# OpenDriveLab/ViDAR

Measured on AMD Instinct MI355X. Metric: train samples/sec (6-cam->BEV step), higher is better.
Workload: dtype f32

## Files before the change

include/vidar_hip.h:

```cpp
#ifndef VIDAR_HIP_H_
#define VIDAR_HIP_H_

#include <stddef.h>
#include <stdint.h>

#ifdef __cplusplus
extern "C" {
#endif

#define VIDAR_ERR_BAD_ARG (-22)

int vidar_abi_version(void);
int vidar_marker(int id, void* stream);

int vidar_set_deterministic(int on);
int vidar_get_deterministic(void);

int vidar_dvr_max_d(void);

int vidar_dvr_render_forward_f32(const float* sigma, const float* origin, const float* points,
                                 const float* tindex, float* pred_dist ,
                                 float* gt_dist , int N, int M, int T, int TO, int Z, int Y,
                                 int X, int train_phase, void* stream);

int vidar_dvr_render_f32(const float* sigma, const float* origin, const float* points,
                         const float* tindex, float* pred_dist, float* gt_dist, float* grad_sigma,
                         int N, int M, int T, int TO, int Z, int Y, int X, int loss_type,
                         void* stream);

int vidar_dvr_init_f32(const float* points, const float* tindex, float* occupancy, int N, int M,
                       int T, int Z, int Y, int X, void* stream);

int vidar_dvxlr_max_d(void);


int vidar_dvr_set_sort_min_waves(int min_waves);
int vidar_dvr_set_traversal(int mode);
int vidar_dvxlr_set_pad_mode(int mode);

int vidar_dvxlr_render_f32(const float* sigma, const float* origin, const float* points,
                           const float* tindex, float* pred_dist, float* gt_dist, float* dd_dsigma,
                           float* indices, int N, int M, int T, int TO, int Z, int Y, int X,
                           void* stream);

size_t vidar_dvxlr_get_grad_sigma_workspace_bytes(int N, int T, int Z, int Y, int X, int volumes );
int vidar_dvxlr_get_grad_sigma_f32(const float* elementwise_mult ,
                                   const float* indices , const float* tindex,
                                   float* grad_sigma , int N, int M, int L, int T,
                                   int Z, int Y, int X, void* workspace, size_t workspace_bytes,
                                   void* stream);

int vidar_dvxlr2_render_f32(const float* sigma, const float* origin, const float* points,
                            const float* tindex, const float* sigma_regul, float* pred_dist,
                            float* gt_dist, float* dd_dsigma, float* indices, float* ray_pred,
                            float* indicator, int N, int M, int T, int TO, int Z, int Y, int X,
                            void* stream);

int vidar_dvxlr2_get_grad_sigma_f32(const float* elementwise_mult, const float* indices,
                                    const float* tindex, const float* indicator,
                                    const float* grad_ray_pred, float* grad_sigma,
                                    float* grad_sigma_regul, int N, int M, int L, int T, int Z, int Y,
                                    int X, void* workspace, size_t workspace_bytes, void* stream);

size_t vidar_knn1_d3_workspace_bytes(int N, int P1);
int vidar_knn1_d3_fwd(const float* p1, const float* p2, const int64_t* lengths1,
                      const int64_t* lengths2, int64_t* idx, float* dist2, void* workspace, int N,
                      int P1, int P2, void* stream);
int vidar_knn1_d3_bwd(const float* p1, const float* p2, const int64_t* lengths1,
                      const int64_t* lengths2, const int64_t* idx, const float* grad_dist2,
                      float* grad_p1, float* grad_p2, int N, int P1, int P2, void* stream);
int vidar_knn1_d3_bwd_workspace_bytes(int N, int P2, int64_t* bytes);
int vidar_knn1_d3_bwd_ws(const float* p1, const float* p2, const int64_t* lengths1,
                         const int64_t* lengths2, const int64_t* idx, const float* grad_dist2,
                         float* grad_p1, float* grad_p2, int N, int P1, int P2, void* workspace,
                         size_t workspace_bytes, void* stream);

int vidar_msda_fwd_f32(const float* value, const int64_t* spatial_shapes,
                       const int64_t* level_start_index, const float* sampling_loc,
                       const float* attn_weight, float* out, int B, int Nv, int H, int C, int Nq,
                       int L, int P, void* stream);
size_t vidar_msda_bwd_workspace_bytes(int B, int Nv, int H, int Nq, int L, int P);
int vidar_msda_set_item_order(int head_major);
int vidar_msda_bwd_f32(const float* value, const int64_t* spatial_shapes,
                       const int64_t* level_start_index, const float* sampling_loc,
                       const float* attn_weight, const float* grad_out, float* grad_value,
                       float* grad_sampling_loc, float* grad_attn_weight, int B, int Nv, int H, int C,
                       int Nq, int L, int P, void* workspace, size_t workspace_bytes, void* stream);

int vidar_msda_fused_fwd_f32(const float* value, const int64_t* spatial_shapes,
                             const int64_t* level_start_index, const float* off_raw, const float* logit_raw,
                             const float* ref, float* loc_out, float* w_out, float* out, int bs, int Qn, int Nv,
                             int H, int C, int Nq, int L, int P, int R, int mode, int merge_queue, void* stream);
int vidar_msda_fused_bwd_f32(const float* value, const int64_t* spatial_shapes,
                             const int64_t* level_start_index, const float* sampling_loc,
                             const float* attn_weight, const float* grad_out, float* grad_value,
                             float* grad_off_raw, float* grad_logit_raw, int bs, int Qn, int Nv, int H, int C,
                             int Nq, int L, int P, int merge_queue, void* workspace, size_t workspace_bytes, void* stream);

int vidar_drop_add_ln_fwd_f32(const float* x, const float* residual, const float* gamma, const float* beta, float* y,
                              float* sum_out, float* mean_out, float* rstd_out, int64_t rows, int C, float p, float eps,
                              uint32_t seed, void* stream);
int vidar_drop_add_ln_bwd_f32(const float* grad_y, const float* sum_in, const float* gamma, const float* mean_in,
                              const float* rstd_in, float* grad_x, float* grad_residual, float* grad_gamma,
                              float* grad_beta, void* workspace, int64_t rows, int C, float p, uint32_t seed,
                              void* stream);
size_t vidar_drop_add_ln_bwd_workspace_bytes(int64_t rows);

int vidar_relu_drop_fwd_f32(const float* x, float* y, int64_t n, float p, uint32_t seed, void* stream);
int vidar_relu_drop_bwd_f32(const float* grad_y, const float* y, float* grad_x, int64_t n, float p, void* stream);

int vidar_colsum_f32(const float* x, float* out, int64_t rows, int cols, void* stream);

int vidar_sca_plan_f32(const float* ref_3d, const float* lidar2img, float* ref_cam, uint8_t* bev_mask,
                       float* count, int64_t* idx, uint8_t* valid, int32_t* lens, int32_t* slot_of,
                       const float* pc_range, float img_h, float img_w, int F, int B, int N, int Q, int D,
                       void* stream);
int vidar_sca_rows_f32(const float* src, const int64_t* idx, const uint8_t* valid, const float* count, float* dst,
                       int B, int N, int S, int stride, int Q, int C, void* stream);
int vidar_sca_combine_f32(const float* src, const int32_t* slot_of, const float* count, float* dst, int B, int N,
                          int S, int Q, int C, void* stream);

size_t vidar_latent_render_bwd_workspace_bytes(int bs, int H, int W, int Z, int maps );
int vidar_latent_render_prob_fwd_f32(const float* occ, float* path_prob, int bs, int H, int W, int Z,
                                     int grid_num, float step, int act, void* stream);
int vidar_latent_render_prob_bwd_f32(const float* occ, const float* grad_path_prob, float* grad_occ,
                                     int bs, int H, int W, int Z, int grid_num, float step, int act,
                                     void* workspace, size_t workspace_bytes, void* stream);
int vidar_latent_render_gather_fwd_f32(const float* path_prob, const float* lora_a, float* feat,
                                       float* msum, int bs, int H, int W, int Z, int grid_num,
                                       float step, float eps, void* stream);
int vidar_latent_render_gather_bwd_f32(const float* path_prob, const float* lora_a, const float* feat,
                                       const float* msum, const float* grad_feat,
                                       float* grad_path_prob, float* grad_lora_a, int bs, int H,
                                       int W, int Z, int grid_num, float step, float eps,
                                       void* workspace, size_t workspace_bytes, void* stream);
int vidar_latent_render_gather_grouped_fwd_f32(const float* path_prob, const float* lora_a, float* feat, float* msum,
                                               int bs, int H, int W, int Z, int A, int grid_num, float step,
                                               float eps, void* stream);
int vidar_latent_render_gather_grouped_bwd_f32(const float* path_prob, const float* lora_a, const float* feat,
                                               const float* msum, const float* grad_feat, float* grad_path_prob,
                                               float* grad_lora_a, int bs, int H, int W, int Z, int A, int grid_num,
                                               float step, float eps, void* workspace, size_t workspace_bytes,
                                               void* stream);

size_t vidar_ray_bwd_workspace_bytes(int F, int Z, int Y, int X);
int vidar_ray_ce_fwd_f32(const float* sigma, const float* origin, const float* gt_pts,
                         const float* tindex, float* ce, float* lse, float* valid, int F, int R,
                         int Z, int Y, int X, int K, float step, void* stream);
int vidar_ray_ce_bwd_f32(const float* sigma, const float* origin, const float* gt_pts,
                         const float* tindex, const float* lse, const float* grad_ce,
                         float* grad_sigma, int F, int R, int Z, int Y, int X, int K, float step,
                         void* workspace, size_t workspace_bytes, void* stream);
int vidar_ray_gumbel_fwd_f32(const float* sigma, const float* origin, const float* pts,
                             const float* tindex, const float* noise , float* dist,
                             float* aux , int F, int R, int Z, int Y, int X, int K,
                             float step, void* stream);
int vidar_ray_gumbel_bwd_f32(const float* sigma, const float* origin, const float* pts,
                             const float* tindex, const float* aux, const float* grad_dist,
                             float* grad_sigma, int F, int R, int Z, int Y, int X, int K, float step,
                             void* workspace, size_t workspace_bytes, void* stream);
int vidar_ray_argmax_f32(const float* sigma, const float* origin, const float* pts,
                         const float* tindex, float* pred_dist, float* gt_dist, int F, int R, int Z,
                         int Y, int X, int K, float step, void* stream);
int vidar_ray_dist_fwd_f32(const float* sigma, const float* origin, const float* gt_pts,
                           const float* tindex, const float* noise , float* dist,
                           float* gt_len, float* aux , float* valid, int F, int R, int Z,
                           int Y, int X, int K, float step, void* stream);
int vidar_ray_dist_bwd_f32(const float* sigma, const float* origin, const float* gt_pts,
                           const float* tindex, const float* aux, const float* grad_dist,
                           float* grad_sigma, int F, int R, int Z, int Y, int X, int K, float step,
                           void* workspace, size_t workspace_bytes, void* stream);
int vidar_ray_max_k(void);
int vidar_ray_force_streamed(int on);

#define VIDAR_GEMM_F32 0
#define VIDAR_GEMM_BF16X3 1
#define VIDAR_GEMM_K_MAJOR 0
#define VIDAR_GEMM_MN_MAJOR 1
int vidar_gemm_f32(const float* A, int64_t lda, int a_layout, const float* B, int64_t ldb, int b_layout, float* C,
                   int64_t ldc, int M, int N, int K, int batch, int64_t strideA, int64_t strideB, int64_t strideC,
                   const float* scale, const float* shift, int vec_axis, const float* residual, int64_t ldr,
                   int64_t strideR, int relu, int precision, int reduce, float* a_rowsum, void* workspace,
                   size_t workspace_bytes, void* stream);
int vidar_gemm_splits(int M, int N, int K, int batch, int precision, int reduce);
size_t vidar_gemm_workspace_bytes(int M, int N, int K, int batch, int precision, int reduce);
int vidar_gemm_set_variant(int variant);

int vidar_dcn_set_variant(int variant);
int vidar_dcn_im2col_f32(const float* x, const float* offset, const float* mask, float* cols, int N,
                         int C, int H, int W, int Ho, int Wo, int kh, int kw, int stride, int pad,
                         int dil, void* stream);
int vidar_dcn_col2im_det_workspace_bytes(int N, int C, int H, int W, int64_t* bytes);
int vidar_dcn_col2im_f32(const float* grad_cols, const float* x, const float* offset,
                         const float* mask, float* grad_x, float* grad_offset, float* grad_mask,
                         int N, int C, int H, int W, int Ho, int Wo, int kh, int kw, int stride,
                         int pad, int dil, void* workspace, size_t workspace_bytes, void* stream);
size_t vidar_dcn_col2im_workspace_bytes(int N, int H, int W, int Ho, int Wo, int kh, int kw);

size_t vidar_conv3x3_few_workspace_bytes(int C);
int vidar_conv3x3_few_f32(const float* x, const float* weight, const float* bias, float* out, int N, int C, int H, int W,
                          int Cout, void* workspace, size_t workspace_bytes, void* stream);

int vidar_affine_act_fwd_f32(const float* x, const float* scale, const float* shift,
                             const float* residual, float* y, int N, int C, int HW, int relu,
                             void* stream);
int vidar_stem_bn_relu_pool_f32(const float* x, const float* scale, const float* shift, float* y, int N, int C,
                                int H, int W, void* stream);
int vidar_affine_act_bwd_f32(const float* grad_y, const float* y, const float* scale, float* grad_x,
                             float* grad_residual, int N, int C, int HW, int relu, void* stream);

int vidar_dcnv3_set_variant(int variant);
int vidar_dcnv3_forward_f32(const float* input, const float* offset, const float* mask, float* out, int N, int H, int W,
                            int kh, int kw, int stride_h, int stride_w, int pad_h, int pad_w, int dil_h, int dil_w,
                            int group, int group_channels, float offset_scale, void* stream);
size_t vidar_dcnv3_backward_workspace_bytes(int N, int H, int W, int kh, int kw, int stride_h, int stride_w, int pad_h,
                                            int pad_w, int dil_h, int dil_w, int group, int group_channels);
int vidar_dcnv3_backward_f32(const float* input, const float* offset, const float* mask, const float* grad_out,
                             float* grad_input, float* grad_offset, float* grad_mask, int N, int H, int W, int kh, int kw,
                             int stride_h, int stride_w, int pad_h, int pad_w, int dil_h, int dil_w, int group,
                             int group_channels, float offset_scale, void* workspace, size_t workspace_bytes, void* stream);

int vidar_det_match_cost_f32(const float* cls, const float* box, const float* gt_box_norm, const int32_t* gt_label,
                             const int32_t* gt_start, float* cost, float alpha, float gamma, float cls_weight,
                             float reg_weight, int NL, int B, int Q, int C, int total_g, void* stream);
size_t vidar_det_loss_workspace_bytes(int NL, int B, int Q);
int vidar_det_loss_fwd_f32(const float* cls, const float* box, const int32_t* labels, const int32_t* matched_gt,
                           const float* gt_box_norm, const int32_t* gt_start, const float* code_weights, float* sums,
                           float alpha, float gamma, int NL, int B, int Q, int C, int total_g, void* workspace,
                           size_t workspace_bytes, void* stream);
int vidar_det_loss_bwd_f32(const float* cls, const float* box, const int32_t* labels, const int32_t* matched_gt,
                           const float* gt_box_norm, const int32_t* gt_start, const float* code_weights,
                           const float* grad_sums, float* grad_cls, float* grad_box, float alpha, float gamma, int NL,
                           int B, int Q, int C, int total_g, void* stream);

int vidar_det_assign_workspace_bytes(int NL, int B, int Q, int total_g, int64_t* bytes);
int vidar_det_assign_f32(const float* cost, const int32_t* gt_start, int32_t* matched, int32_t* status, int NL, int B,
                         int Q, int total_g, void* workspace, size_t workspace_bytes, void* stream);

int vidar_det_eval_match_f32(const float* pred_box, const int32_t* pred_attr, const int32_t* pred_start,
                             const float* gt_box, const int32_t* gt_attr, const int32_t* gt_start, const float* dist_ths,
                             int32_t* match, int32_t* gt_match, float* err, int P, int G, int NS, int NT, int tp_index,
                             int num_classes, int barrier_class, void* stream);

int vidar_ray_eval_workspace_bytes(int P, int64_t* bytes);
int vidar_ray_eval_f64(const float* pred, const int32_t* pred_start, const float* gt, const int32_t* gt_start,
                       const float* origin, void* partial, int32_t* nn_idx, void* ray_err, void* interp, int P, int G,
                       int S, int max_gt, void* workspace, size_t workspace_bytes, void* stream);

#define VIDAR_IMG_PHOTO_FLOATS 12
int vidar_img_photometric_u8(const uint8_t* src, const float* photo, uint8_t* dst, int n, int H, int W, void* stream);
int vidar_img_photometric_f32(const uint8_t* src, const float* photo, float* dst, int n, int H, int W, void* stream);
size_t vidar_img_resample_workspace_bytes(int n, int crop_h, int out_w);
int vidar_img_resample_u8(const uint8_t* src, uint8_t* dst, int n, int H, int W, int crop_x, int crop_y, int crop_w,
                          int crop_h, int out_w, int out_h, const int32_t* tab_x, int ksize_x, const int32_t* tab_y,
                          int ksize_y, int flip, void* workspace, size_t workspace_bytes, void* stream);
int vidar_img_normalise_f32(const uint8_t* src, const float* photo, float* dst, int n, int H, int W, int out_h, int out_w,
                            int Hp, int Wp, const float* mean, const float* stdv, int to_rgb, void* stream);

#ifdef __cplusplus
}
#endif
#endif
```

vidar_amd/_lib.py:

```python
from __future__ import annotations

import ctypes
import os
from pathlib import Path

_PKG = Path(__file__).resolve().parent
LIB_PATH = _PKG / "libvidar_hip.so"
_lib = None
BAD_ARG = -22


class VidarHipError(RuntimeError):
    pass


def lib() -> ctypes.CDLL:
    global _lib
    if _lib is None:
        import torch
        if not LIB_PATH.exists():
            raise VidarHipError(
                f"{LIB_PATH} not found: build it with `python -m vidar_amd.build` "
                f"(or __graft_entry__.build()); vidar_amd has no CPU fallback")
        _lib = declare(ctypes.CDLL(str(LIB_PATH)))
        dcn = os.environ.get("VIDAR_DCN_VARIANT")
        if dcn is not None:
            _lib.vidar_dcn_set_variant(int(dcn))
        v3 = os.environ.get("VIDAR_DCNV3_VARIANT")
        if v3 is not None:
            _lib.vidar_dcnv3_set_variant(int(v3))
        order = os.environ.get("VIDAR_MSDA_ITEM_ORDER")
        if order is not None:
            _lib.vidar_msda_set_item_order(int(order))
    return _lib


_KIND = {"p": ctypes.c_void_p, "i": ctypes.c_int, "l": ctypes.c_int64, "z": ctypes.c_size_t, "f": ctypes.c_float,
         "u": ctypes.c_uint32}
_ABI = {
    "vidar_abi_version": "i",
    "vidar_marker": "i i p",
    "vidar_set_deterministic": "i i",
    "vidar_get_deterministic": "i",
    "vidar_dvr_max_d": "i",
    "vidar_dvr_render_forward_f32": "i 6p 8i p",
    "vidar_dvr_render_f32": "i 7p 8i p",
    "vidar_dvr_init_f32": "i 3p 6i p",
    "vidar_dvxlr_max_d": "i",
    "vidar_dvr_set_sort_min_waves": "i i",
    "vidar_dvr_set_traversal": "i i",
    "vidar_dvxlr_set_pad_mode": "i i",
    "vidar_dvxlr_render_f32": "i 8p 7i p",
    "vidar_dvxlr_get_grad_sigma_workspace_bytes": "z 6i",
    "vidar_dvxlr_get_grad_sigma_f32": "i 4p 7i p z p",
    "vidar_dvxlr2_render_f32": "i 11p 7i p",
    "vidar_dvxlr2_get_grad_sigma_f32": "i 7p 7i p z p",
    "vidar_knn1_d3_workspace_bytes": "z 2i",
    "vidar_knn1_d3_fwd": "i 7p 3i p",
    "vidar_knn1_d3_bwd": "i 8p 3i p",
    "vidar_knn1_d3_bwd_workspace_bytes": "i 2i p",
    "vidar_knn1_d3_bwd_ws": "i 8p 3i p z p",
    "vidar_msda_fwd_f32": "i 6p 7i p",
    "vidar_msda_bwd_workspace_bytes": "z 6i",
    "vidar_msda_set_item_order": "i i",
    "vidar_msda_bwd_f32": "i 9p 7i p z p",
    "vidar_msda_fused_fwd_f32": "i 9p 11i p",
    "vidar_msda_fused_bwd_f32": "i 9p 9i p z p",
    "vidar_drop_add_ln_fwd_f32": "i 8p l i 2f u p",
    "vidar_drop_add_ln_bwd_f32": "i 10p l i f u p",
    "vidar_drop_add_ln_bwd_workspace_bytes": "z l",
    "vidar_relu_drop_fwd_f32": "i 2p l f u p",
    "vidar_relu_drop_bwd_f32": "i 3p l f p",
    "vidar_colsum_f32": "i 2p l i p",
    "vidar_sca_plan_f32": "i 10p 2f 5i p",
    "vidar_sca_rows_f32": "i 5p 6i p",
    "vidar_sca_combine_f32": "i 4p 5i p",
    "vidar_latent_render_bwd_workspace_bytes": "z 5i",
    "vidar_latent_render_prob_fwd_f32": "i 2p 5i f i p",
    "vidar_latent_render_prob_bwd_f32": "i 3p 5i f i p z p",
    "vidar_latent_render_gather_fwd_f32": "i 4p 5i 2f p",
    "vidar_latent_render_gather_bwd_f32": "i 7p 5i 2f p z p",
    "vidar_latent_render_gather_grouped_fwd_f32": "i 4p 6i 2f p",
    "vidar_latent_render_gather_grouped_bwd_f32": "i 7p 6i 2f p z p",
    "vidar_ray_bwd_workspace_bytes": "z 4i",
    "vidar_ray_ce_fwd_f32": "i 7p 6i f p",
    "vidar_ray_ce_bwd_f32": "i 7p 6i f p z p",
    "vidar_ray_gumbel_fwd_f32": "i 7p 6i f p",
    "vidar_ray_gumbel_bwd_f32": "i 7p 6i f p z p",
    "vidar_ray_argmax_f32": "i 6p 6i f p",
    "vidar_ray_dist_fwd_f32": "i 9p 6i f p",
    "vidar_ray_dist_bwd_f32": "i 7p 6i f p z p",
    "vidar_ray_max_k": "i",
    "vidar_ray_force_streamed": "i i",
    "vidar_gemm_f32": "i p l i p l i p l 4i 3l 2p i p 2l 3i 2p z p",
    "vidar_gemm_splits": "i 6i",
    "vidar_gemm_workspace_bytes": "z 6i",
    "vidar_gemm_set_variant": "i i",
    "vidar_dcn_set_variant": "i i",
    "vidar_dcn_im2col_f32": "i 4p 11i p",
    "vidar_dcn_col2im_f32": "i 7p 11i p z p",
    "vidar_dcn_col2im_workspace_bytes": "z 7i",
    "vidar_dcn_col2im_det_workspace_bytes": "i 4i p",
    "vidar_conv3x3_few_workspace_bytes": "z i",
    "vidar_conv3x3_few_f32": "i 4p 5i p z p",
    "vidar_affine_act_fwd_f32": "i 5p 4i p",
    "vidar_stem_bn_relu_pool_f32": "i 4p 4i p",
    "vidar_affine_act_bwd_f32": "i 5p 4i p",
    "vidar_dcnv3_set_variant": "i i",
    "vidar_dcnv3_forward_f32": "i 4p 13i f p",
    "vidar_dcnv3_backward_workspace_bytes": "z 13i",
    "vidar_dcnv3_backward_f32": "i 7p 13i f p z p",
    "vidar_det_match_cost_f32": "i 6p 4f 5i p",
    "vidar_det_loss_workspace_bytes": "z 3i",
    "vidar_det_loss_fwd_f32": "i 8p 2f 5i p z p",
    "vidar_det_loss_bwd_f32": "i 10p 2f 5i p",
    "vidar_det_assign_workspace_bytes": "i 4i p",
    "vidar_det_assign_f32": "i 4p 4i p z p",
    "vidar_det_eval_match_f32": "i 10p 7i p",
    "vidar_ray_eval_workspace_bytes": "i i p",
    "vidar_ray_eval_f64": "i 9p 4i p z p",
    "vidar_img_photometric_u8": "i 3p 3i p",
    "vidar_img_photometric_f32": "i 3p 3i p",
    "vidar_img_resample_workspace_bytes": "z 3i",
    "vidar_img_resample_u8": "i 2p 9i p i p 2i p z p",
    "vidar_img_normalise_f32": "i 3p 7i 2p i p",
}


def signature(name):
    ret, *runs = _ABI[name].split()
    return _KIND[ret], [_KIND[r[-1]] for r in runs for _ in range(int(r[:-1] or 1))]


def declare(cdll):
    for name in _ABI:
        try:
            fn = getattr(cdll, name)
        except AttributeError:
            raise VidarHipError(f"{name} is not exported by {cdll._name}: rebuild the library") from None
        fn.restype, fn.argtypes = signature(name)
    return cdll


def check(rc: int, what: str):
    if rc == 0:
        return
    if rc == BAD_ARG:
        raise ValueError(f"{what}: invalid argument")
    raise VidarHipError(f"{what}: HIP error {rc}")


def ptr(t):
    return None if t is None else t.data_ptr()


def workspace(nbytes_fn, *dims, like):
    import torch
    n = nbytes_fn(*dims)
    if n == 0:
        return None, None, 0
    ws = torch.empty(n, dtype=torch.uint8, device=like.device)
    return ws, ptr(ws), n


def stream_of(t):
    import torch
    return torch.cuda.current_stream(t.device).cuda_stream


class OpTimer:
    def __init__(self):
        self.enabled = False
        self.records = {}

    def reset(self):
        self.records = {}

    class _Span:
        __slots__ = ("t", "name", "nbytes", "e0")

        def __init__(self, t, name, nbytes):
            self.t, self.name, self.nbytes = t, name, nbytes

        def __enter__(self):
            import torch
            self.e0 = torch.cuda.Event(enable_timing=True)
            self.e0.record()

        def __exit__(self, *exc):
            import torch
            e1 = torch.cuda.Event(enable_timing=True)
            e1.record()
            self.t.records.setdefault(self.name, []).append((self.e0, e1, self.nbytes))

    class _Null:
        def __enter__(self): return None
        def __exit__(self, *exc): return False

    _null = _Null()

    def span(self, name, nbytes=0):
        return OpTimer._Span(self, name, nbytes) if self.enabled else OpTimer._null

    def summary(self):
        import torch
        torch.cuda.synchronize()
        out = {}
        for name, recs in self.records.items():
            ms = [a.elapsed_time(b) for a, b, _ in recs]
            out[name] = dict(calls=len(ms), total_ms=sum(ms), avg_ms=sum(ms) / len(ms),
                             bytes_per_call=sum(r[2] for r in recs) / len(recs))
        return out


TIMER = OpTimer()
```

vidar_amd/plugin/backbones.py:

```python
from __future__ import annotations

import ctypes
import math
import os

import torch
import torch.nn as nn
import torch.nn.functional as F
from torch.autograd import Function
from torch.autograd.function import once_differentiable

from .registry import BACKBONES, NECKS
from .._lib import lib, check, ptr, stream_of, workspace, TIMER
from .. import gemm as G
from .. import deterministic


def dcn_col2im(grad_cols, x, offset, mask, kh, kw, stride, pad, dil, Ho, Wo, gather=True):
    N, C, H, W = x.shape
    gx = torch.empty_like(x); goff = torch.empty_like(offset); gm = torch.empty_like(mask)
    if deterministic.sync():
        nbytes = ctypes.c_int64(0)
        check(lib().vidar_dcn_col2im_det_workspace_bytes(N, C, H, W, ctypes.addressof(nbytes)), "dcn_col2im")
        nbytes = nbytes.value
        ws = torch.empty(nbytes, dtype=torch.uint8, device=x.device)
        ws_ptr = ptr(ws)
    else:
        ws, ws_ptr, nbytes = workspace(lib().vidar_dcn_col2im_workspace_bytes, N, H, W, Ho, Wo, kh, kw, like=x) \
            if gather else (None, None, 0)
    with TIMER.span("dcn_col2im", 4 * (3 * x.numel() + 2 * offset.numel() + 2 * mask.numel() + grad_cols.numel())):
        check(lib().vidar_dcn_col2im_f32(ptr(grad_cols), ptr(x), ptr(offset), ptr(mask), ptr(gx), ptr(goff), ptr(gm),
                                         N, C, H, W, Ho, Wo, kh, kw, stride, pad, dil, ws_ptr, nbytes, stream_of(x)),
              "dcn_col2im")
    return gx, goff, gm


class _ModulatedDeformConv(Function):

    @staticmethod
    def forward(ctx, x, offset, mask, weight, bias, stride, pad, dil, gemm_mode="lib", scale=None, shift=None,
                relu=False):
        x, offset, mask = x.float().contiguous(), offset.float().contiguous(), mask.float().contiguous()
        N, C, H, W = x.shape
        Cout, _, kh, kw = weight.shape
        Ho = (H + 2 * pad - dil * (kh - 1) - 1) // stride + 1
        Wo = (W + 2 * pad - dil * (kw - 1) - 1) // stride + 1
        cols = torch.empty((N, C * kh * kw, Ho * Wo), device=x.device)
        with TIMER.span("dcn_im2col", 4 * (x.numel() + offset.numel() + mask.numel() + cols.numel())):
            check(lib().vidar_dcn_im2col_f32(ptr(x), ptr(offset), ptr(mask), ptr(cols), N, C, H, W, Ho,
                                             Wo, kh, kw, stride, pad, dil, stream_of(x)), "dcn_im2col")
        fused = scale is not None
        if gemm_mode == "lib":
            assert not fused
            out = torch.bmm(weight.reshape(1, Cout, -1).expand(N, -1, -1), cols)
            if bias is not None:
                out = out + bias.view(1, -1, 1)
        else:
            sh = shift
            if bias is not None:
                sh = bias.float() if not fused else (shift + bias.float() * scale)
            out = G.conv_forward(weight.reshape(Cout, -1), cols, scale, sh, None, relu, G.precision_of(gemm_mode))
        ctx.save_for_backward(x, offset, mask, weight, cols, scale, out if (fused and relu) else None)
        ctx.cfg = (stride, pad, dil, Ho, Wo, bias is not None, gemm_mode, fused, relu)
        return out.view(N, Cout, Ho, Wo)

    @staticmethod
    @once_differentiable
    def backward(ctx, grad_out):
        x, offset, mask, weight, cols, scale, y = ctx.saved_tensors
        stride, pad, dil, Ho, Wo, has_bias, gemm_mode, fused, relu = ctx.cfg
        N, C, H, W = x.shape
        Cout, _, kh, kw = weight.shape
        go = grad_out.float().contiguous().view(N, Cout, Ho * Wo)
        if fused:
            go = _affine_act_backward(go, y if relu else go, scale, relu, False)[0]
        if gemm_mode == "lib":
            grad_weight = torch.bmm(go, cols.transpose(1, 2)).sum(0).reshape(weight.shape)
            grad_cols = torch.bmm(weight.reshape(1, Cout, -1).transpose(1, 2).expand(N, -1, -1), go)
        else:
            prec = G.precision_of(gemm_mode)
            grad_weight = G.conv_grad_weight(go, cols, prec).reshape(weight.shape) if ctx.needs_input_grad[3] else None
            grad_cols = G.conv_grad_input(weight.reshape(Cout, -1), go, prec)
        gx, goff, gm = dcn_col2im(grad_cols, x, offset, mask, kh, kw, stride, pad, dil, Ho, Wo)
        return (gx, goff, gm, grad_weight, (go.sum((0, 2)) if has_bias else None), None, None, None, None, None, None,
                None)


def modulated_deform_conv2d(x, offset, mask, weight, bias=None, stride=1, padding=0, dilation=1, bn=None, relu=False):
    m = G.mode() if (x.is_cuda and G.own_kernels()) else "lib"
    scale = shift = None
    if bn is not None:
        assert m != "lib"
        scale, shift = bn._scale_shift()
    return _ModulatedDeformConv.apply(x, offset, mask, weight, bias, int(stride), int(padding), int(dilation), m,
                                      scale, shift, bool(relu))


_CONV_OFFSET_OWN = os.environ.get("VIDAR_CONV_OFFSET", "lib") == "own"


class _Conv3x3Few(Function):

    @staticmethod
    def forward(ctx, x, weight, bias):
        x = x.contiguous()
        w = weight.contiguous()
        N, C, H, W = x.shape
        Cout = w.shape[0]
        out = torch.empty((N, Cout, H, W), device=x.device, dtype=torch.float32)
        ws, ws_ptr, ws_bytes = workspace(lib().vidar_conv3x3_few_workspace_bytes, C, like=x)
        with TIMER.span("conv3x3_few", 4 * (x.numel() + out.numel())):
            check(lib().vidar_conv3x3_few_f32(ptr(x), ptr(w), ptr(bias), ptr(out), N, C, H, W, Cout, ws_ptr, ws_bytes,
                                              stream_of(x)), "conv3x3_few")
        ctx.save_for_backward(x, w)
        ctx.has_bias = bias is not None
        return out

    @staticmethod
    @once_differentiable
    def backward(ctx, g):
        x, w = ctx.saved_tensors
        need = [ctx.needs_input_grad[0], ctx.needs_input_grad[1], ctx.has_bias and ctx.needs_input_grad[2]]
        gx, gw, gb = torch.ops.aten.convolution_backward(g.contiguous(), x, w, [w.shape[0]] if ctx.has_bias else None,
                                                         [1, 1], [1, 1], [1, 1], False, [0, 0], 1, need)
        return gx, gw, gb


def conv3x3_few_ok(conv, x):
    return (_CONV_OFFSET_OWN and x.is_cuda and x.dtype == torch.float32 and conv.weight.dtype == torch.float32
            and not torch.is_autocast_enabled() and x.dim() == 4
            and conv.kernel_size == (3, 3) and conv.stride == (1, 1) and conv.padding == (1, 1) and conv.dilation == (1, 1)
            and conv.groups == 1 and conv.padding_mode == "zeros" and conv.out_channels <= 32 and conv.in_channels % 8 == 0
            and x.shape[3] <= 191 and x.shape[2] * x.shape[3] < (1 << 30) and x.numel() > 0)


class ModulatedDeformConv2dPack(nn.Module):

    def __init__(self, in_channels, out_channels, kernel_size, stride=1, padding=0, dilation=1,
                 groups=1, deform_groups=1, bias=True):
        super().__init__()
        if groups != 1 or deform_groups != 1:
            raise NotImplementedError("DCNv2 kernels are built for groups == deform_groups == 1")
        k = kernel_size
        self.stride, self.padding, self.dilation, self.k = stride, padding, dilation, k
        self.weight = nn.Parameter(torch.empty(out_channels, in_channels, k, k))
        self.bias = nn.Parameter(torch.zeros(out_channels)) if bias else None
        n = in_channels * k * k
        nn.init.uniform_(self.weight, -1.0 / math.sqrt(n), 1.0 / math.sqrt(n))
        self.conv_offset = nn.Conv2d(in_channels, 3 * k * k, k, stride, padding, dilation, bias=True)
        nn.init.zeros_(self.conv_offset.weight)
        nn.init.zeros_(self.conv_offset.bias)

    def forward(self, x, bn=None, relu=False):
        if conv3x3_few_ok(self.conv_offset, x):
            out = _Conv3x3Few.apply(x, self.conv_offset.weight, self.conv_offset.bias)
        else:
            out = self.conv_offset(x)
        o1, o2, mask = torch.chunk(out, 3, dim=1)
        offset = torch.cat((o1, o2), dim=1)
        fuse = dict(bn=bn, relu=relu) if bn is not None else {}
        return modulated_deform_conv2d(x, offset, torch.sigmoid(mask), self.weight, self.bias,
                                       self.stride, self.padding, self.dilation, **fuse)


class _AffineAct(Function):

    @staticmethod
    def forward(ctx, x, scale, shift, residual, relu):
        x = x.float().contiguous()
        N, C, H, W = x.shape
        res = residual.float().contiguous() if residual is not None else None
        y = torch.empty_like(x)
        with TIMER.span("affine_act_fwd", 4 * x.numel() * (3 if res is not None else 2)):
            check(lib().vidar_affine_act_fwd_f32(ptr(x), ptr(scale), ptr(shift), ptr(res), ptr(y), N, C,
                                                 H * W, int(relu), stream_of(x)), "affine_act_fwd")
        ctx.save_for_backward(y, scale)
        ctx.cfg = (relu, residual is not None)
        return y

    @staticmethod
    @once_differentiable
    def backward(ctx, gy):
        y, scale = ctx.saved_tensors
        relu, has_res = ctx.cfg
        gx, gres = _affine_act_backward(gy.float().contiguous(), y, scale, relu, has_res)
        return gx, None, None, gres, None


def _affine_act_backward(gy, y, scale, relu, has_res):
    N, C = y.shape[:2]
    HW = y.numel() // (N * C)
    gx = torch.empty_like(y)
    gres = torch.empty_like(y) if has_res else None
    with TIMER.span("affine_act_bwd", 4 * y.numel() * (4 if has_res else 3)):
        check(lib().vidar_affine_act_bwd_f32(ptr(gy), ptr(y), ptr(scale), ptr(gx), ptr(gres), N, C,
                                             HW, int(relu), stream_of(y)), "affine_act_bwd")
    return gx, gres


class FrozenBN(nn.BatchNorm2d):

    def __init__(self, c, requires_grad=False):
        super().__init__(c)
        for p in self.parameters():
            p.requires_grad = requires_grad
        self._cache = None

    def _scale_shift(self):
        key = (self.weight._version, self.bias._version, self.running_mean._version,
               self.running_var._version, self.weight.device)
        if self._cache is None or self._cache[0] != key:
            with torch.no_grad():
                scale = (self.weight / torch.sqrt(self.running_var + self.eps)).float().contiguous()
                shift = (self.bias - self.running_mean * scale).float().contiguous()
            self._cache = (key, scale, shift)
        return self._cache[1], self._cache[2]

    def forward(self, x, residual=None, relu=False):
        if self.weight.requires_grad or not x.is_cuda:
            y = F.batch_norm(x, self.running_mean, self.running_var, self.weight, self.bias, False, 0.0,
                             self.eps)
            if residual is not None:
                y = y + residual
            return F.relu(y, inplace=True) if relu else y
        scale, shift = self._scale_shift()
        return _AffineAct.apply(x, scale, shift, residual, relu)


def stem_bn_relu_pool(x, bn):
    if not x.is_cuda or bn.weight.requires_grad or (torch.is_grad_enabled() and x.requires_grad):
        return None
    x = x.float().contiguous()
    N, C, H, W = x.shape
    if W % 4 or N * C > 65535:
        return None
    scale, shift = bn._scale_shift()
    y = torch.empty((N, C, (H - 1) // 2 + 1, W // 2), device=x.device, dtype=torch.float32)
    with TIMER.span("stem_bn_relu_pool", 4 * (x.numel() + y.numel())):
        check(lib().vidar_stem_bn_relu_pool_f32(ptr(x), ptr(scale), ptr(shift), ptr(y), N, C, H, W, stream_of(x)),
              "stem_bn_relu_pool")
    return y


class Conv1x1(nn.Conv2d):
    as_gemm = os.environ.get("VIDAR_CONV1X1_GEMM", "1") != "0"
    any_device = False

    def gemm_form(self, x):
        return (self.as_gemm and (x.is_cuda or self.any_device) and self.kernel_size == (1, 1) and self.padding == (0, 0)
                and self.groups == 1)

    def forward(self, x, presampled=False):
        if not self.gemm_form(x):
            assert not presampled
            return super().forward(x)
        if self.stride != (1, 1) and not presampled:
            x = x[:, :, ::self.stride[0], ::self.stride[1]].contiguous()
        N, C, H, W = x.shape
        out = torch.bmm(self.weight.view(1, self.out_channels, C).expand(N, -1, -1), x.reshape(N, C, H * W))
        if self.bias is not None:
            out = out + self.bias.view(1, -1, 1)
        return out.view(N, self.out_channels, H, W)


_AUTO_FUSE_RES = os.environ.get("VIDAR_AUTO_FUSE_RES", "1") != "0"


class _Conv1x1Identity(Function):

    @staticmethod
    def forward(ctx, x, weight):
        N, C, H, W = x.shape
        Cout = weight.shape[0]
        out = torch.bmm(weight.view(1, Cout, C).expand(N, -1, -1), x.reshape(N, C, H * W))
        ctx.save_for_backward(x, weight)
        return out.view(N, Cout, H, W), x.view_as(x)

    @staticmethod
    @once_differentiable
    def backward(ctx, g_out, g_ident):
        x, weight = ctx.saved_tensors
        N, C, H, W = x.shape
        Cout = weight.shape[0]
        gx = gw = None
        if g_out is None:
            return g_ident, None
        go = g_out.contiguous().view(N, Cout, H * W)
        if ctx.needs_input_grad[0]:
            wt = weight.view(1, Cout, C).transpose(1, 2).expand(N, -1, -1)
            if g_ident is not None:
                gx = g_ident.contiguous().view(N, C, H * W).baddbmm_(wt, go).view(N, C, H, W)
            else:
                gx = torch.bmm(wt, go).view(N, C, H, W)
        if ctx.needs_input_grad[1]:
            gw = torch.bmm(go, x.reshape(N, C, H * W).transpose(1, 2)).sum(0).view_as(weight)
        return gx, gw


_SHORTCUT_ACCUMULATE = os.environ.get("VIDAR_SHORTCUT_ACCUMULATE", "1") != "0"


def conv1x1_with_identity_ok(conv, x):
    return (_SHORTCUT_ACCUMULATE and isinstance(conv, Conv1x1) and conv.gemm_form(x) and conv.stride == (1, 1)
            and conv.bias is None and x.dtype == torch.float32 and conv.weight.dtype == torch.float32
            and x.requires_grad and torch.is_grad_enabled() and not torch.is_autocast_enabled() and x.is_contiguous())


class _Conv1x1BNAct(Function):

    @staticmethod
    def forward(ctx, x, weight, scale, shift, residual, relu, precision):
        x = x.float().contiguous()
        N, C, H, W = x.shape
        Cout = weight.shape[0]
        res = residual.float().contiguous().view(N, Cout, H * W) if residual is not None else None
        y = G.conv_forward(weight.reshape(Cout, C), x.view(N, C, H * W), scale, shift, res, relu, precision)
        ctx.save_for_backward(x, weight, scale, y if relu else None)
        ctx.cfg = (relu, residual is not None, precision)
        return y.view(N, Cout, H, W)

    @staticmethod
    @once_differentiable
    def backward(ctx, gy):
        x, weight, scale, y = ctx.saved_tensors
        relu, has_res, precision = ctx.cfg
        N, C, H, W = x.shape
        Cout = weight.shape[0]
        gy = gy.float().contiguous().view(N, Cout, H * W)
        gz, gres = _affine_act_backward(gy, y if relu else gy, scale, relu, has_res)
        gx = G.conv_grad_input(weight.reshape(Cout, C), gz, precision).view(N, C, H, W) if ctx.needs_input_grad[0] else None
        gw = G.conv_grad_weight(gz, x.view(N, C, H * W), precision).view_as(weight) if ctx.needs_input_grad[1] else None
        return gx, gw, None, None, (gres.view(N, Cout, H, W) if has_res else None), None, None


def _fuses_1x1(conv, bn, x, residual, hw, m):
    fuse = G.own_kernels(m) or (m == "auto" and residual is not None and _AUTO_FUSE_RES)
    in_range = 0 < hw < (1 << 22) and max(conv.in_channels, conv.out_channels) * hw < (1 << 29)
    return (fuse and x.is_cuda and not bn.weight.requires_grad and conv.bias is None and conv.kernel_size == (1, 1)
            and conv.padding == (0, 0) and conv.groups == 1 and in_range)


def conv1x1_bn_act(conv, bn, x, residual=None, relu=False, presampled=False):
    if presampled:
        return _conv1x1_bn_act_presampled(conv, bn, x, residual, relu)
    m = G.mode()
    hw = ((x.shape[2] - 1) // conv.stride[0] + 1) * ((x.shape[3] - 1) // conv.stride[1] + 1) if x.dim() == 4 else 0
    if not _fuses_1x1(conv, bn, x, residual, hw, m):
        return bn(conv(x), residual=residual, relu=relu)
    if conv.stride != (1, 1):
        x = x[:, :, ::conv.stride[0], ::conv.stride[1]]
    scale, shift = bn._scale_shift()
    return _Conv1x1BNAct.apply(x, conv.weight, scale, shift, residual, bool(relu), G.precision_of(m))


def _conv1x1_bn_act_presampled(conv, bn, xs, residual, relu):
    m = G.mode()
    if not _fuses_1x1(conv, bn, xs, residual, xs.shape[2] * xs.shape[3] if xs.dim() == 4 else 0, m):
        return bn(conv(xs, presampled=True), residual=residual, relu=relu)
    scale, shift = bn._scale_shift()
    return _Conv1x1BNAct.apply(xs, conv.weight, scale, shift, residual, bool(relu), G.precision_of(m))


_SHARE_SUBSAMPLE = os.environ.get("VIDAR_SHARE_SUBSAMPLE", "1") != "0"


class Bottleneck(nn.Module):
    expansion = 4

    def __init__(self, inplanes, planes, stride=1, downsample=None, style="caffe", dcn=None, bn_grad=False):
        super().__init__()
        s1, s2 = (stride, 1) if style == "caffe" else (1, stride)
        self.conv1 = Conv1x1(inplanes, planes, 1, stride=s1, bias=False)
        self.bn1 = FrozenBN(planes, bn_grad)
        if dcn is not None:
            self.conv2 = ModulatedDeformConv2dPack(planes, planes, 3, stride=s2, padding=1, dilation=1,
                                                   deform_groups=dcn.get("deform_groups", 1), bias=False)
        else:
            self.conv2 = nn.Conv2d(planes, planes, 3, stride=s2, padding=1, bias=False)
        self.bn2 = FrozenBN(planes, bn_grad)
        self.conv3 = Conv1x1(planes, planes * 4, 1, bias=False)
        self.bn3 = FrozenBN(planes * 4, bn_grad)
        self.downsample = downsample

    def _shares_subsample(self, x):
        d = self.downsample
        return (_SHARE_SUBSAMPLE and d is not None and len(d) == 2 and isinstance(d[0], Conv1x1) and isinstance(d[1], FrozenBN)
                and self.conv1.stride != (1, 1) and d[0].stride == self.conv1.stride
                and self.conv1.gemm_form(x) and d[0].gemm_form(x))

    def forward(self, x):
        if self._shares_subsample(x):
            sh, sw = self.conv1.stride
            xs = x[:, :, ::sh, ::sw].contiguous()
            identity = conv1x1_bn_act(self.downsample[0], self.downsample[1], xs, presampled=True)
            out = conv1x1_bn_act(self.conv1, self.bn1, xs, relu=True, presampled=True)
            return self._tail(out, identity)
        if self.downsample is None:
            identity = x
            if conv1x1_with_identity_ok(self.conv1, x) and not _fuses_1x1(self.conv1, self.bn1, x, None,
                                                                            x.shape[2] * x.shape[3], G.mode()):
                out, identity = _Conv1x1Identity.apply(x, self.conv1.weight)
                return self._tail(self.bn1(out, relu=True), identity)
        elif len(self.downsample) == 2 and isinstance(self.downsample[1], FrozenBN):
            identity = conv1x1_bn_act(self.downsample[0], self.downsample[1], x)
        else:
            identity = self.downsample(x)
        out = conv1x1_bn_act(self.conv1, self.bn1, x, relu=True)
        return self._tail(out, identity)

    def _tail(self, out, identity):
        if (isinstance(self.conv2, ModulatedDeformConv2dPack) and G.own_kernels() and out.is_cuda
                and not self.bn2.weight.requires_grad):
            out = self.conv2(out, bn=self.bn2, relu=True)
        else:
            out = self.bn2(self.conv2(out), relu=True)
        return conv1x1_bn_act(self.conv3, self.bn3, out, residual=identity, relu=True)


@BACKBONES.register_module()
class ResNet(nn.Module):
    arch = {50: (3, 4, 6, 3), 101: (3, 4, 23, 3), 152: (3, 8, 36, 3)}

    def __init__(self, depth=101, num_stages=4, out_indices=(0, 1, 2, 3), frozen_stages=-1,
                 norm_cfg=dict(type="BN", requires_grad=True), norm_eval=True, style="pytorch", dcn=None,
                 stage_with_dcn=(False, False, False, False), strides=(1, 2, 2, 2), in_channels=3,
                 base_channels=64, init_cfg=None, pretrained=None, **kwargs):
        super().__init__()
        if dcn is not None and dcn.get("type") != "DCNv2":
            raise NotImplementedError(dcn)
        bn_grad = norm_cfg.get("requires_grad", True)
        self.out_indices, self.frozen_stages, self.norm_eval = out_indices, frozen_stages, norm_eval
        self.conv1 = nn.Conv2d(in_channels, base_channels, 7, stride=2, padding=3, bias=False)
        self.bn1 = FrozenBN(base_channels, bn_grad)
        inplanes = base_channels
        self.res_layers = []
        for i, nblocks in enumerate(self.arch[depth][:num_stages]):
            planes = base_channels * 2 ** i
            stage_dcn = dcn if stage_with_dcn[i] else None
            down = None
            if strides[i] != 1 or inplanes != planes * 4:
                down = nn.Sequential(Conv1x1(inplanes, planes * 4, 1, stride=strides[i], bias=False),
                                     FrozenBN(planes * 4, bn_grad))
            blocks = [Bottleneck(inplanes, planes, strides[i], down, style, stage_dcn, bn_grad)]
            inplanes = planes * 4
            blocks += [Bottleneck(inplanes, planes, 1, None, style, stage_dcn, bn_grad) for _ in range(1, nblocks)]
            name = f"layer{i + 1}"
            self.add_module(name, nn.Sequential(*blocks))
            self.res_layers.append(name)
        self._freeze_stages()

    def _freeze_stages(self):
        if self.frozen_stages >= 0:
            for m in (self.conv1, self.bn1):
                for p in m.parameters():
                    p.requires_grad = False
        for i in range(1, self.frozen_stages + 1):
            for p in getattr(self, f"layer{i}").parameters():
                p.requires_grad = False

    def forward(self, x):
        x = self.conv1(x)
        y = stem_bn_relu_pool(x, self.bn1)
        x = y if y is not None else F.max_pool2d(self.bn1(x, relu=True), 3, stride=2, padding=1)
        outs = []
        for i, name in enumerate(self.res_layers):
            x = getattr(self, name)(x)
            if i in self.out_indices:
                outs.append(x)
        return tuple(outs)


class _ConvModule(nn.Module):

    def __init__(self, cin, cout, k, stride=1, padding=0):
        super().__init__()
        self.conv = nn.Conv2d(cin, cout, k, stride=stride, padding=padding)
        nn.init.xavier_uniform_(self.conv.weight)
        nn.init.zeros_(self.conv.bias)

    def forward(self, x):
        return self.conv(x)


@NECKS.register_module()
class FPN(nn.Module):
    def __init__(self, in_channels, out_channels, num_outs, start_level=0, end_level=-1,
                 add_extra_convs=False, relu_before_extra_convs=False, init_cfg=None, **kwargs):
        super().__init__()
        self.start_level = start_level
        self.backbone_end_level = len(in_channels) if end_level == -1 else end_level
        self.num_outs = num_outs
        self.add_extra_convs = "on_input" if add_extra_convs is True else add_extra_convs
        self.relu_before_extra_convs = relu_before_extra_convs
        self.lateral_convs = nn.ModuleList()
        self.fpn_convs = nn.ModuleList()
        for i in range(start_level, self.backbone_end_level):
            self.lateral_convs.append(_ConvModule(in_channels[i], out_channels, 1))
            self.fpn_convs.append(_ConvModule(out_channels, out_channels, 3, padding=1))
        extra = num_outs - (self.backbone_end_level - start_level)
        if self.add_extra_convs and extra >= 1:
            for i in range(extra):
                cin = in_channels[self.backbone_end_level - 1] if (i == 0 and self.add_extra_convs == "on_input") else out_channels
                self.fpn_convs.append(_ConvModule(cin, out_channels, 3, stride=2, padding=1))

    def forward(self, inputs):
        lat = [l(inputs[i + self.start_level]) for i, l in enumerate(self.lateral_convs)]
        for i in range(len(lat) - 1, 0, -1):
            lat[i - 1] = lat[i - 1] + F.interpolate(lat[i], size=lat[i - 1].shape[2:], mode="nearest")
        outs = [self.fpn_convs[i](lat[i]) for i in range(len(lat))]
        if self.num_outs > len(outs):
            if not self.add_extra_convs:
                for _ in range(self.num_outs - len(outs)):
                    outs.append(F.max_pool2d(outs[-1], 1, stride=2))
            else:
                if self.add_extra_convs == "on_input":
                    src = inputs[self.backbone_end_level - 1]
                elif self.add_extra_convs == "on_lateral":
                    src = lat[-1]
                else:
                    src = outs[-1]
                outs.append(self.fpn_convs[len(lat)](src))
                for i in range(len(lat) + 1, self.num_outs):
                    outs.append(self.fpn_convs[i](F.relu(outs[-1]) if self.relu_before_extra_convs else outs[-1]))
        return tuple(outs)
```

Baseline: 2.934.

## Fuse ResNet stem 7x7 conv with BN, ReLU and maxpool in one MFMA kernel

Adds a HIP kernel that computes the frozen ResNet stem (7x7 stride-2 conv, 3->64 channels) with MFMA f32 instructions from an LDS input window, then applies BN scale/shift, ReLU and the 3x3 stride-2 max pool in registers before writing the pooled output. The aim is to avoid writing and re-reading the full-resolution conv output and to drop the separate conv launch. It runs only when the stem is frozen and no gradients are needed. The hand-written conv may be slower than the vendor conv for some shapes, and its summation order differs from the library conv.

```diff
diff --git a/include/vidar_hip.h b/include/vidar_hip.h
--- a/include/vidar_hip.h
+++ b/include/vidar_hip.h
@@ -208,6 +208,9 @@
                                 int H, int W, void* stream);
 int vidar_affine_act_bwd_f32(const float* grad_y, const float* y, const float* scale, float* grad_x,
                              float* grad_residual, int N, int C, int HW, int relu, void* stream);
+int vidar_stem_conv_bn_relu_pool_f32(const float* x, const float* w, const float* scale, const float* shift, float* y,
+                                     int N, int Cin, int H, int W, int Cout, int ksize, int stride, int pad,
+                                     void* stream);
 
 int vidar_dcnv3_set_variant(int variant);
 int vidar_dcnv3_forward_f32(const float* input, const float* offset, const float* mask, float* out, int N, int H, int W,
diff --git a/vidar_amd/_lib.py b/vidar_amd/_lib.py
--- a/vidar_amd/_lib.py
+++ b/vidar_amd/_lib.py
@@ -106,6 +106,7 @@
     "vidar_affine_act_fwd_f32": "i 5p 4i p",
     "vidar_stem_bn_relu_pool_f32": "i 4p 4i p",
     "vidar_affine_act_bwd_f32": "i 5p 4i p",
+    "vidar_stem_conv_bn_relu_pool_f32": "i 5p 8i p",
     "vidar_dcnv3_set_variant": "i i",
     "vidar_dcnv3_forward_f32": "i 4p 13i f p",
     "vidar_dcnv3_backward_workspace_bytes": "z 13i",
diff --git a/vidar_amd/csrc/stem_conv.hip b/vidar_amd/csrc/stem_conv.hip
--- /dev/null
+++ b/vidar_amd/csrc/stem_conv.hip
@@ -0,0 +1,202 @@
+#include "vidar_common.h"
+#include "vidar_hip.h"
+
+namespace {
+
+constexpr int THREADS = 512;
+constexpr int CIN = 3, COUT = 64, KS = 7, KTOT = CIN * KS * KS, KSTEPS = (KTOT + 1) / 2;
+constexpr int TC = 31;
+constexpr int WR = 4;
+constexpr int RGROUPS = THREADS / 128;
+constexpr int TR = RGROUPS * WR;
+constexpr int CROWS = 2 * WR + 1;
+constexpr int Q = 34;
+constexpr int ROW = 4 * Q;
+constexpr int WIN_ROWS = 4 * TR + 7;
+constexpr int WIN_COLS = 4 * TC + 9;
+constexpr int WIN = WIN_ROWS * CIN * ROW;
+constexpr int WL = KSTEPS * 2 * COUT;
+constexpr int LDS_BYTES = (WIN + WL + 2 * COUT) * (int)sizeof(float);
+#ifndef VIDAR_STEM_BATCH
+#define VIDAR_STEM_BATCH 8
+#endif
+constexpr int BATCH = VIDAR_STEM_BATCH;
+
+typedef float f32x16 __attribute__((ext_vector_type(16)));
+
+#ifndef VIDAR_STEM_ABL
+#define VIDAR_STEM_ABL 0
+#endif
+constexpr int ABL = VIDAR_STEM_ABL;
+
+constexpr int PAIRED = 70, HALF_SEGS = 10, LAST_SEG = 20;
+__host__ __device__ constexpr int step_seg(int s, int h) { return s < PAIRED ? s / KS + HALF_SEGS * h : LAST_SEG; }
+__host__ __device__ constexpr int step_col(int s, int h) { return s < PAIRED ? s % KS : 2 * (s - PAIRED) + h; }
+__host__ __device__ constexpr int step_weight(int s, int h) {
+  const int seg = step_seg(s, h), j = step_col(s, h);
+  return j >= KS ? -1 : (seg % CIN) * KS * KS + (seg / CIN) * KS + j;
+}
+__host__ __device__ constexpr int col_offset(int j, int e) { return ((j + 2 * e) & 3) * Q + ((j + 2 * e) >> 2); }
+
+__device__ inline float relu_nan(float v) { return v < 0.0f ? 0.0f : v; }
+__device__ inline float max_nan(float a, float b) { return (a > b || a != a) ? a : b; }
+
+struct StemArgs {
+  const float* x; const float* w; const float* scale; const float* shift; float* y;
+  int H, W, Hc, Wc, Hp, Wp, tiles_x, tiles_y, total;
+};
+
+__global__ __launch_bounds__(THREADS, 4) void stem_conv_pool_kernel(StemArgs g) {
+  extern __shared__ float lds[];
+  float* win = lds;
+  float* wl = lds + WIN;
+  float* bn = wl + WL;
+  const int tid = threadIdx.x, lane = tid & 63, wave = tid >> 6, l31 = lane & 31, h = lane >> 5;
+  const int ch = wave & 1, rh = wave >> 1;
+  const int H = g.H, W = g.W, Hc = g.Hc, Wc = g.Wc, Hp = g.Hp, Wp = g.Wp;
+
+  if (tid < 2 * COUT) bn[tid] = tid < COUT ? g.scale[tid] : g.shift[tid - COUT];
+  for (int e = tid; e < WL; e += THREADS) {
+    const int o = e & (COUT - 1), sh = e / COUT, k = step_weight(sh >> 1, sh & 1);
+    wl[e] = k < 0 ? 0.0f : g.w[o * KTOT + k];
+  }
+  const float* wa = wl + h * COUT + 32 * ch + l31;
+  const float ninf = -__builtin_inff();
+
+  for (int t = blockIdx.x; t < g.total; t += gridDim.x) {
+    const int n = t / (g.tiles_x * g.tiles_y), rem = t - n * (g.tiles_x * g.tiles_y);
+    const int ty = rem / g.tiles_x, tx = rem - ty * g.tiles_x;
+    const int hp0 = ty * TR, p0 = tx * TC;
+    const int y0 = 4 * hp0 - 5, x0 = 4 * p0 - 5;
+    const float* xn = g.x + (int64_t)n * CIN * H * W;
+
+    __syncthreads();
+    if (!(ABL & 1)) {
+      for (int e0 = 0; e0 < WIN; e0 += THREADS * BATCH) {
+        float v[BATCH];
+#pragma unroll
+        for (int u = 0; u < BATCH; ++u) {
+          const int e = e0 + tid + THREADS * u;
+          const int rc = e / ROW, xw = e - rc * ROW, r = rc / CIN, c = rc - r * CIN;
+          const int gy = y0 + r, gx = x0 + xw;
+          const bool ok = e < WIN && xw < WIN_COLS && gy >= 0 && gy < H && gx >= 0 && gx < W;
+          const float ld = xn[ok ? (c * H + gy) * W + gx : 0];
+          v[u] = ok ? ld : 0.0f;
+        }
+#pragma unroll
+        for (int u = 0; u < BATCH; ++u) {
+          const int e = e0 + tid + THREADS * u;
+          const int rc = e / ROW, xw = e - rc * ROW;
+          if (e < WIN) win[rc * ROW + (xw & 3) * Q + (xw >> 2)] = v[u];
+        }
+      }
+    }
+    __syncthreads();
+
+    const int hpw = hp0 + WR * rh;
+    if (hpw >= Hp) continue;
+    const int wp = p0 + l31;
+    const bool vo = 2 * wp - 1 >= 0 && 2 * wp - 1 < Wc, ve = 2 * wp < Wc;
+    const bool st = l31 < TC && wp < Wp;
+    float* yn = g.y + (int64_t)n * COUT * Hp * Wp + wp;
+    float vm[16];
+#pragma unroll 1
+    for (int q = 0; q < CROWS; ++q) {
+      const int cy = 2 * hpw - 1 + q;
+      const int hp = hpw + ((q + 1) >> 1) - 1;
+      if (q && hp >= Hp) break;
+      float hrow[16];
+      if (cy >= 0 && cy < Hc) {
+        f32x16 acc_o, acc_e;
+#pragma unroll
+        for (int r = 0; r < 16; ++r) { acc_o[r] = 0.0f; acc_e[r] = 0.0f; }
+        if (!(ABL & 2)) {
+          const float* wb = win + (4 * WR * rh + 2 * q) * (CIN * ROW) + l31;
+          const float* wbh = wb + h * (HALF_SEGS * ROW);
+#pragma unroll
+          for (int s = 0; s < KSTEPS; ++s) {
+            float bo, be;
+            if (s < PAIRED) {
+              bo = wbh[step_seg(s, 0) * ROW + col_offset(step_col(s, 0), 0)];
+              be = wbh[step_seg(s, 0) * ROW + col_offset(step_col(s, 0), 1)];
+            } else {
+              const int j0 = step_col(s, 0), j1 = step_col(s, 1) < KS ? step_col(s, 1) : j0;
+              bo = wb[LAST_SEG * ROW + (h ? col_offset(j1, 0) : col_offset(j0, 0))];
+              be = wb[LAST_SEG * ROW + (h ? col_offset(j1, 1) : col_offset(j0, 1))];
+              if (step_col(s, 1) >= KS) { bo = h ? 0.0f : bo; be = h ? 0.0f : be; }
+            }
+            const float a = wa[s * 2 * COUT];
+            acc_o = __builtin_amdgcn_mfma_f32_32x32x2f32(a, bo, acc_o, 0, 0, 0);
+            acc_e = __builtin_amdgcn_mfma_f32_32x32x2f32(a, be, acc_e, 0, 0, 0);
+          }
+        }
+#pragma unroll
+        for (int r = 0; r < 16; ++r) {
+          const int o = 32 * ch + (r & 3) + 8 * (r >> 2) + 4 * h;
+          const float sc = bn[o], sh = bn[COUT + o];
+          float vo_ = relu_nan(__builtin_fmaf(acc_o[r], sc, sh)), ve_ = relu_nan(__builtin_fmaf(acc_e[r], sc, sh));
+          if (ABL & 4) { hrow[r] = vo_ + ve_; continue; }
+          vo_ = vo ? vo_ : ninf;
+          ve_ = ve ? ve_ : ninf;
+          const float nb = __shfl_down(vo_, 1, 32);
+          hrow[r] = max_nan(max_nan(vo_, ve_), nb);
+        }
+      } else {
+#pragma unroll
+        for (int r = 0; r < 16; ++r) hrow[r] = ninf;
+      }
+      if (q == 0) {
+#pragma unroll
+        for (int r = 0; r < 16; ++r) vm[r] = hrow[r];
+      } else if (q & 1) {
+#pragma unroll
+        for (int r = 0; r < 16; ++r) vm[r] = max_nan(vm[r], hrow[r]);
+      } else {
+#pragma unroll
+        for (int r = 0; r < 16; ++r) {
+          const int o = 32 * ch + (r & 3) + 8 * (r >> 2) + 4 * h;
+          if (st) yn[(o * Hp + hp) * Wp] = max_nan(vm[r], hrow[r]);
+          vm[r] = hrow[r];
+        }
+      }
+    }
+  }
+}
+
+int device_cus() {
+  static int cus = 0;
+  if (cus == 0) {
+    int dev = 0, n = 0;
+    cus = (hipGetDevice(&dev) == hipSuccess &&
+           hipDeviceGetAttribute(&n, hipDeviceAttributeMultiprocessorCount, dev) == hipSuccess && n > 0) ? n : 256;
+  }
+  return cus;
+}
+
+}
+
+extern "C" int vidar_stem_conv_bn_relu_pool_f32(const float* x, const float* w, const float* scale, const float* shift,
+                                                float* y, int N, int Cin, int H, int W, int Cout, int ksize, int stride,
+                                                int pad, void* stream) {
+  VIDAR_ENTER();
+  if (N < 0 || H <= 0 || W <= 0) return VIDAR_ERR_BAD_ARG;
+  if (Cin != CIN || Cout != COUT || ksize != KS || stride != 2 || pad != 3) return VIDAR_ERR_BAD_ARG;
+  const int Hc = (H - 1) / 2 + 1, Wc = (W - 1) / 2 + 1, Hp = (Hc - 1) / 2 + 1, Wp = (Wc - 1) / 2 + 1;
+  const int64_t lim = (int64_t)1 << 31;
+  if ((int64_t)N * CIN * H * W >= lim || (int64_t)N * COUT * Hp * Wp >= lim) return VIDAR_ERR_BAD_ARG;
+  if (N == 0) return 0;
+  StemArgs g;
+  g.x = x; g.w = w; g.scale = scale; g.shift = shift; g.y = y;
+  g.H = H; g.W = W; g.Hc = Hc; g.Wc = Wc; g.Hp = Hp; g.Wp = Wp;
+  g.tiles_x = (Wp + TC - 1) / TC;
+  g.tiles_y = (Hp + TR - 1) / TR;
+  const int64_t total = (int64_t)N * g.tiles_x * g.tiles_y;
+  if (total >= lim) return VIDAR_ERR_BAD_ARG;
+  g.total = (int)total;
+  static const bool lds_ok = hipFuncSetAttribute(reinterpret_cast<const void*>(stem_conv_pool_kernel),
+                                                 hipFuncAttributeMaxDynamicSharedMemorySize, LDS_BYTES) == hipSuccess;
+  if (!lds_ok) return vidar_last_error();
+  const int grid = g.total < device_cus() ? g.total : device_cus();
+  hipLaunchKernelGGL(stem_conv_pool_kernel, dim3(grid), dim3(THREADS), LDS_BYTES, (hipStream_t)stream, g);
+  return vidar_last_error();
+}
diff --git a/vidar_amd/plugin/backbones.py b/vidar_amd/plugin/backbones.py
--- a/vidar_amd/plugin/backbones.py
+++ b/vidar_amd/plugin/backbones.py
@@ -239,6 +239,35 @@
     with TIMER.span("stem_bn_relu_pool", 4 * (x.numel() + y.numel())):
         check(lib().vidar_stem_bn_relu_pool_f32(ptr(x), ptr(scale), ptr(shift), ptr(y), N, C, H, W, stream_of(x)),
               "stem_bn_relu_pool")
+    return y
+
+
+_STEM_CONV_OWN = os.environ.get("VIDAR_STEM_CONV", "own") == "own"
+
+
+def stem_conv_fused_ok(conv, bn, x, on_device=None):
+    if not _STEM_CONV_OWN:
+        return False
+    if not (x.is_cuda if on_device is None else on_device) or bn.weight.requires_grad:
+        return False
+    if torch.is_grad_enabled() and (x.requires_grad or conv.weight.requires_grad):
+        return False
+    return (conv.bias is None and conv.weight.dtype == torch.float32 and x.dtype == torch.float32 and x.dim() == 4
+            and tuple(conv.weight.shape) == (64, 3, 7, 7) and x.shape[1] == 3
+            and tuple(conv.stride) == (2, 2) and tuple(conv.padding) == (3, 3) and tuple(conv.dilation) == (1, 1)
+            and conv.groups == 1 and conv.padding_mode == "zeros")
+
+
+def stem_conv_bn_relu_pool(x, weight, scale, shift, stride=2, padding=3):
+    if not (x.is_contiguous() and weight.is_contiguous()) or x.dim() != 4 or weight.dim() != 4 or weight.shape[2] != weight.shape[3]:
+        raise ValueError("stem_conv_bn_relu_pool: invalid argument")
+    N, C, H, W = x.shape
+    Hc, Wc = (H - 1) // 2 + 1, (W - 1) // 2 + 1
+    y = torch.empty((N, weight.shape[0], (Hc - 1) // 2 + 1, (Wc - 1) // 2 + 1), device=x.device, dtype=torch.float32)
+    with TIMER.span("stem_conv_bn_relu_pool", 4 * (x.numel() + y.numel())):
+        check(lib().vidar_stem_conv_bn_relu_pool_f32(ptr(x), ptr(weight), ptr(scale), ptr(shift), ptr(y), N, C, H, W,
+                                                     weight.shape[0], weight.shape[2], stride, padding, stream_of(x)),
+              "stem_conv_bn_relu_pool")
     return y
 
 
@@ -459,9 +488,12 @@
                 p.requires_grad = False
 
     def forward(self, x):
-        x = self.conv1(x)
-        y = stem_bn_relu_pool(x, self.bn1)
-        x = y if y is not None else F.max_pool2d(self.bn1(x, relu=True), 3, stride=2, padding=1)
+        if stem_conv_fused_ok(self.conv1, self.bn1, x):
+            x = stem_conv_bn_relu_pool(x.contiguous(), self.conv1.weight.contiguous(), *self.bn1._scale_shift())
+        else:
+            x = self.conv1(x)
+            y = stem_bn_relu_pool(x, self.bn1)
+            x = y if y is not None else F.max_pool2d(self.bn1(x, relu=True), 3, stride=2, padding=1)
         outs = []
         for i, name in enumerate(self.res_layers):
             x = getattr(self, name)(x)
```

New measurement: 2.952 (median of 6 runs). No clear change (+0.6%).
